# telespazio-tim/karios

Hardware: AMD Instinct MI355X
Metric: Mpixels/sec (+ matched keypoints/sec), Sentinel-2 10980^2 pair, KLT + ZNCC (higher is better)
Workload: dtype u8/i32 stencils, f32 LK solve, f64 stretch + ZNCC; 1 GPU; BASELINE config 2: 4 distinct S2-sized pairs 10980x10980 u16 resident in HBM, one per step, 4 per batched submissio...; distinct_pairs_resident=4, contexts=1, klt=Laplacian k=7, maxCorners 20000, one tile, ZNCC of rows with score >= 0.4, parallelism=1 rank(s), each a stream of independent band pairs

## Files before the change

include/karios_hip.h:

```cpp
#ifndef KARIOS_HIP_H
#define KARIOS_HIP_H

#include <stddef.h>
#include <stdint.h>

#ifdef __cplusplus
extern "C" {
#endif

typedef struct km_ctx km_ctx;

enum { KM_U8 = 0, KM_U16 = 1, KM_I16 = 2, KM_F32 = 3, KM_F64 = 4, KM_I32 = 5, KM_U32 = 6 };

enum {
    KM_OK = 0,
    KM_E_ARG = -1,
    KM_E_HIP = -2,
    KM_E_NOMEM = -3,
    KM_E_UNSUPPORTED = -4,
    KM_E_NO_DEVICE = -5,
    KM_E_INTERNAL = -6,
    KM_E_NO_CONVERGENCE = -7,
    KM_E_CAPACITY = -8
};
// ... 27 lines not shown
#define KM_PATH_STAGE_FALLBACK 2
#define KM_PATH_SECOND_PASS 4
#define KM_PATH_PREFIX_GROWN 8
#define KM_PATH_SPEC_RETRY 16
#define KM_PATH_MM_EARLY 32

int km_version(void);
int km_ctx_create(int device, km_ctx **out);
int km_ctx_destroy(km_ctx *ctx);
const char *km_last_error(km_ctx *ctx);
int km_ctx_sync(km_ctx *ctx);
int km_set_profiling(km_ctx *ctx, int enable);
int km_set_option(km_ctx *ctx, const char *name, int value);
int km_is_dev_build(void);
int km_dev_counters(km_ctx *ctx, unsigned long long out[2]);
int km_get_stage_ms(km_ctx *ctx, float *out, int cap, int *n);
const char *km_stage_name(int i);
int km_get_klt_stats(km_ctx *ctx, km_klt_stats *out);

int km_dev_alloc(km_ctx *ctx, size_t bytes, void **dptr);
int km_dev_free(km_ctx *ctx, void *dptr);
int km_h2d(km_ctx *ctx, void *dst_dev, const void *src_host, size_t bytes);
int km_d2h(km_ctx *ctx, void *dst_host, const void *src_dev, size_t bytes);
int km_host_alloc(km_ctx *ctx, size_t bytes, void **hptr);
int km_host_free(km_ctx *ctx , void *hptr);
int km_upload_async(km_ctx *ctx, void *dst_dev, size_t dst_pitch, const void *src_host, size_t src_pitch,
                    size_t width_bytes, size_t rows);
int km_upload_wait(km_ctx *ctx);
int km_upload_check_stats(km_ctx *ctx, int64_t *armed, int64_t *missed);
int km_upload_mark(km_ctx *ctx, int *ticket);
// ... 246 lines not shown
```

karios_amd/_lib.py:

```python
from __future__ import annotations

import ctypes as C
import os
import threading

import numpy as np

_HERE = os.path.dirname(os.path.abspath(__file__))
LIB_PATH = os.environ.get("KARIOS_HIP_LIB") or os.path.join(_HERE, "libkarios_hip.so")

KM_U8, KM_U16, KM_I16, KM_F32 = 0, 1, 2, 3
_DTYPES = {np.dtype("uint8"): KM_U8, np.dtype("uint16"): KM_U16, np.dtype("int16"): KM_I16,
           np.dtype("float32"): KM_F32}


class KariosHipError(RuntimeError):

    code = None


class KltParams(C.Structure):
    _fields_ = [("max_corners", C.c_int32), ("block_size", C.c_int32), ("win_size", C.c_int32),
                ("max_level", C.c_int32), ("max_count", C.c_int32), ("ksize_mon", C.c_int32),
                ("ksize_ref", C.c_int32), ("invert_mon", C.c_int32), ("quality_level", C.c_double),
# ... 47 lines not shown
ECC_CONVERGED, ECC_SKIPPED, ECC_NO_CONVERGENCE = 0, 1, 2

_vp, _i, _d, _sz, _pd = C.c_void_p, C.c_int, C.c_double, C.c_ssize_t, C.POINTER(C.c_double)
_pi = C.POINTER(C.c_int)

SIGNATURES = {
    "km_version": (_i, []),
    "km_ctx_create": (_i, [_i, C.POINTER(_vp)]),
    "km_ctx_destroy": (_i, [_vp]),
    "km_last_error": (C.c_char_p, [_vp]),
    "km_ctx_sync": (_i, [_vp]),
    "km_set_profiling": (_i, [_vp, _i]),
    "km_set_option": (_i, [_vp, C.c_char_p, _i]),
    "km_is_dev_build": (_i, []),
    "km_dev_counters": (_i, [_vp, C.POINTER(C.c_uint64)]),
    "km_get_stage_ms": (_i, [_vp, C.POINTER(C.c_float), _i, _pi]),
    "km_stage_name": (C.c_char_p, [_i]),
    "km_get_klt_stats": (_i, [_vp, C.POINTER(KltStats)]),
    "km_dev_alloc": (_i, [_vp, C.c_size_t, C.POINTER(_vp)]),
    "km_dev_free": (_i, [_vp, _vp]),
    "km_h2d": (_i, [_vp, _vp, _vp, C.c_size_t]),
    "km_d2h": (_i, [_vp, _vp, _vp, C.c_size_t]),
    "km_host_alloc": (_i, [_vp, C.c_size_t, C.POINTER(_vp)]),
    "km_host_free": (_i, [_vp, _vp]),
    "km_upload_async": (_i, [_vp, _vp, C.c_size_t, _vp, C.c_size_t, C.c_size_t, C.c_size_t]),
    "km_upload_wait": (_i, [_vp]),
    "km_upload_check_stats": (_i, [_vp, C.POINTER(C.c_int64), C.POINTER(C.c_int64)]),
    "km_upload_mark": (_i, [_vp, _pi]),
    "km_upload_join": (_i, [_vp, _i]),
    "km_set_frame_sink": (_i, [_vp, _vp, C.c_size_t]),
# ... 268 lines not shown
        self.check(self.lib.km_get_klt_stats(self.handle, C.byref(s)), "km_get_klt_stats")
        return s

    def set_profiling(self, on: bool):
        self.check(self.lib.km_set_profiling(self.handle, int(bool(on))), "km_set_profiling")

    def upload_check_stats(self):
        a, m = C.c_int64(), C.c_int64()
        self.check(self.lib.km_upload_check_stats(self.handle, C.byref(a), C.byref(m)), "km_upload_check_stats")
        return int(a.value), int(m.value)

    def set_option(self, name: str, value: int):
        self.check(self.lib.km_set_option(self.handle, name.encode(), int(value)), "km_set_option")
        self.__dict__.setdefault("_options", {})[name] = int(value)

    def set_frame_sink(self, ptr: int | None, nbytes: int = 0, pitch: int = 0) -> None:
        self.check(self.lib.km_set_frame_sink_pitch(self.handle, C.c_void_p(ptr) if ptr else None, int(nbytes) if ptr else 0, int(pitch) if ptr else 0),
                   "km_set_frame_sink_pitch")
        self.__dict__["_frame_sink"] = (int(ptr), int(nbytes), int(pitch)) if ptr else (None, 0, 0)

    @property
    def frame_sink(self) -> tuple:
        return self.__dict__.get("_frame_sink", (None, 0, 0))

    def get_option(self, name: str, default: int = 0) -> int:
        return self.__dict__.get("_options", {}).get(name, default)

    def phase_info(self) -> tuple[int, float]:
        path, margin = C.c_int(), C.c_double()
        self.check(self.lib.km_phase_info(self.handle, C.byref(path), C.byref(margin)), "km_phase_info")
# ... 35 lines not shown
```

karios_amd/csrc/api.hip:

```cpp
#include "api_internal.hpp"
#include "fft64_plan.hpp"
#include <vector>

#include <dlfcn.h>

#include <cstdarg>
#include <cstdio>
#include <cstdlib>
#include <cstring>
#include <new>

static thread_local std::string g_last_error;

int km_fail(km_ctx *ctx, int code, const char *fmt, ...)
{
    char buf[1024];
    va_list ap;
    va_start(ap, fmt);
    vsnprintf(buf, sizeof buf, fmt, ap);
    va_end(ap);
    g_last_error = buf;
    if (ctx) ctx->err = buf;
    return code;
}
// ... 130 lines not shown
    if (strcmp(name, "mm_early") == 0) { c->opt_mm_early = value != 0; return KM_OK; }
    if (strcmp(name, "frame_mi") == 0) { c->opt_frame_mi = value != 0; return KM_OK; }
    if (strcmp(name, "frame_clip") == 0) { c->opt_frame_clip = value != 0; return KM_OK; }
    if (strcmp(name, "units_pipeline") == 0) {
        if (!value) { const int rf = km_units_flush(c); if (rf) return rf; }
        c->opt_units_pipeline = value != 0;
        return KM_OK;
    }
    if (strcmp(name, "key_cap") == 0) { c->opt_key_cap = value < 0 ? 0 : value; return KM_OK; }
    if (strcmp(name, "stage_cap") == 0) { c->opt_stage_cap = value < 0 ? 0 : value; return KM_OK; }
    if (strcmp(name, "topk_factor") == 0) { c->opt_topk_factor = value < 0 ? 0 : value; return KM_OK; }
    if (strcmp(name, "select_first") == 0) { c->opt_select_first = value < 0 ? 0 : value; return KM_OK; }
    if (strcmp(name, "stash_cap") == 0) { c->opt_stash_cap = value < 0 ? 0 : value; return KM_OK; }
    if (strcmp(name, "spec_flag") == 0) { c->opt_spec_flag = value < 0 ? 0 : value; return KM_OK; }
    if (strcmp(name, "ransac_first_batch") == 0) { c->opt_ransac_first_batch = value < 0 ? 0 : value; return KM_OK; }
    if (strcmp(name, "defer") == 0) { c->opt_no_defer = value == 0; return KM_OK; }
    if (strcmp(name, "phase_fp64") == 0) { c->opt_phase_fp64 = value != 0; return KM_OK; }
    if (strcmp(name, "fft61") == 0) { c->opt_fft61 = value != 0; return KM_OK; }
    if (strcmp(name, "fft_herm") == 0) { c->opt_fft_herm = value != 0; return KM_OK; }
    if (strcmp(name, "f64_half") == 0) { c->opt_f64_half = value != 0; return KM_OK; }
    if (strcmp(name, "f64_pair") == 0) { c->opt_f64_pair = value != 0; return KM_OK; }
    if (strcmp(name, "f64_plain") == 0) { c->opt_f64_plain = value != 0; return KM_OK; }
    if (strcmp(name, "roctx") == 0) { c->opt_roctx = value != 0; return KM_OK; }
    if (strcmp(name, "profile_every") == 0) { c->opt_profile_every = value < 1 ? 1 : value; return KM_OK; }
    if (strcmp(name, "profile_stage") == 0) { c->opt_profile_stage = (value >= 0 && value < ST_COUNT) ? value : -1; return KM_OK; }
#ifdef KM_DEV
    if (strcmp(name, "fft_cross") == 0) { c->opt_fft_cross_fused = value != 0; return KM_OK; }
    if (strcmp(name, "f64_prime_t") == 0) { c->opt_f64_prime_t = value < 0 ? 0 : value; return KM_OK; }
    if (strcmp(name, "f64_smooth_t") == 0) { c->opt_f64_smooth_t = value < 0 ? 0 : value; return KM_OK; }
    if (strcmp(name, "defer_valid") == 0) { c->opt_defer_valid = value != 0; return KM_OK; }
    if (strcmp(name, "aux_early") == 0) { c->opt_aux_early = value != 0; return KM_OK; }
    if (strcmp(name, "aux_priority") == 0) { c->opt_aux_priority = value != 0; return KM_OK; }
    if (strcmp(name, "eig3_count") == 0) { c->opt_eig3_count = value != 0; return KM_OK; }
    if (strcmp(name, "prep_hist_plain") == 0) { c->opt_prep_plain = value != 0; return KM_OK; }
#endif
    return km_fail(c, KM_E_ARG, "km_set_option: unknown option '%s'", name);
}

int km_dev_counters(km_ctx *c, unsigned long long out[2])
{
#ifdef KM_DEV
    if (!c || !out) return km_fail(c, KM_E_ARG, "km_dev_counters: null argument");
    km_scalars *sc = (km_scalars *)c->ws[WS_SCALARS].p;
    if (!sc) return km_fail(c, KM_E_ARG, "km_dev_counters: no tile call yet");
    unsigned long long h[2];
    { const int rq = km_d2h_queue(c, h, &sc->skip_total, sizeof h); if (rq) return rq; }
    { const int rq = km_d2h_flush(c); if (rq) return rq; }
    out[0] = h[0]; out[1] = h[1];
    return KM_OK;
#else
    (void)out;
    return km_fail(c, KM_E_UNSUPPORTED, "km_dev_counters: development build only");
#endif
// ... 319 lines not shown
```

karios_amd/csrc/api_band.hip:

```cpp
#include "api_internal.hpp"

#include <cstring>
#include <vector>

extern "C" {

int km_minmax_dev(km_ctx *c, const void *d_img, int dtype, int H, int W, ptrdiff_t stride, double out_minmax[2])
{
    int rc;
    if ((rc = begin_call(c)) || (rc = check_image(c, d_img, H, W, stride, "minmax"))) return rc;
    if (!km_dtype_size(dtype) || !out_minmax) return km_fail(c, KM_E_ARG, "minmax: bad dtype %d or null output", dtype);
    km_scalars *sc = scalars(c);
    if (!sc) return KM_E_NOMEM;
    if (dtype == KM_U8) { out_minmax[0] = out_minmax[1] = 0.0; return KM_OK; }
    if ((rc = kd_minmax(c, d_img, dtype, H, W, stride, sc->mm))) return rc;
    KM_D2H(c, out_minmax, sc->mm, 2 * sizeof(double));
    KM_FLUSH(c);
    return KM_OK;
}

int km_band_prefilter_dev(km_ctx *c, const void *d_ref, const void *d_mon, int dtype, int H, int W, ptrdiff_t sref, ptrdiff_t smon,
                          const double minmax[4], const double *nodata_ref, const double *nodata_mon, int ksize_ref, int ksize_mon, int invert_mon,
                          int own_y0, int own_y1, const uint8_t *d_user_mask, uint8_t *d_lap_ref, uint8_t *d_lap_mon, uint8_t *d_mask,
                          int64_t *valid_owned)
{
    int rc;
    if ((rc = begin_call(c)) || (rc = check_image(c, d_ref, H, W, sref, "band_prefilter")) || (rc = check_image(c, d_mon, H, W, smon, "band_prefilter")))
        return rc;
    if (!km_dtype_size(dtype) || !minmax || !d_lap_ref || !d_lap_mon || !d_mask || !valid_owned) return km_fail(c, KM_E_ARG, "band_prefilter: bad arguments");
    if (own_y0 < 0 || own_y1 > H || own_y0 > own_y1) return km_fail(c, KM_E_ARG, "band_prefilter: own rows [%d, %d) outside 0..%d", own_y0, own_y1, H);
    km_scalars *sc = scalars(c);
    if (!sc) return KM_E_NOMEM;
    KM_HIP(c, hipMemsetAsync(sc, 0, sizeof *sc, c->stream));
    { const int rch = h2d_now(c, sc->mm, minmax, 4 * sizeof(double)); if (rch) return rch; }
    if ((rc = kd_stretch_laplacian_pair(c, d_ref, d_mon, dtype, H, W, sref, smon, sc->mm, ksize_ref, ksize_mon, invert_mon, nodata_ref, nodata_mon,
                                        d_lap_ref, d_lap_mon, d_user_mask ? nullptr : d_mask, &sc->valid)))
        return rc;
    if (d_user_mask) KM_HIP(c, hipMemcpyAsync(d_mask, d_user_mask, (size_t)H * W, hipMemcpyDeviceToDevice, c->stream));
    if (own_y0 > 0) KM_HIP(c, hipMemsetAsync(d_mask, 0, (size_t)own_y0 * W, c->stream));
    if (own_y1 < H) KM_HIP(c, hipMemsetAsync(d_mask + (size_t)own_y1 * W, 0, (size_t)(H - own_y1) * W, c->stream));
    KM_HIP(c, hipMemsetAsync(&sc->valid, 0, sizeof sc->valid, c->stream));
    if ((rc = kd_count_nonzero(c, d_mask, (size_t)H * W, &sc->valid))) return rc;
    unsigned long long v = 0;
    KM_D2H(c, &v, &sc->valid, sizeof v);
    KM_FLUSH(c);
    *valid_owned = (int64_t)v;
    return KM_OK;
}

int km_band_eigen_dev(km_ctx *c, const uint8_t *d_lap_ref, const uint8_t *d_mask, int H, int W, int block, double quality, unsigned *local_max_key)
{
    int rc;
// ... 176 lines not shown
```

karios_amd/csrc/common.hpp:

```cpp
#pragma once
#include <hip/hip_runtime.h>
#include <stddef.h>
#include <stdint.h>
#include <stdlib.h>
#include <atomic>
#include <memory>
#include <mutex>
#include <functional>
#include <string>
#include <vector>

#include "../../include/karios_hip.h"

#define KM_WAVE 64
#define KM_NSHARD 16
#define KM_TK_NB 2048
#define KM_UNITS_MAX 16

__host__ __device__ __forceinline__ int km_reflect101(int p, int len)
{
    if ((unsigned)p < (unsigned)len) return p;
    if (len == 1) return 0;
    do {
        p = p < 0 ? -p : 2 * len - 2 - p;
    } while ((unsigned)p >= (unsigned)len);
    return p;
}

enum km_stage {
    ST_MINMAX = 0,
    ST_LAPLACIAN,
// ... 141 lines not shown
    WS_SF_REFINED,
    WS_SF_KP,
    WS_SF_DESC,
    WS_SF_PERM,
    WS_SF_OUT,
    WS_AC_IN,
    WS_AC_COLS,
    WS_AC_BSUM,
    WS_AC_STATE,
    WS_AC_PART,
    WS_AC_FLAG,
    WS_AC_SCAN,
    WS_AC_KEYS0,
    WS_AC_KEYS1,
    WS_CL_COLS,
    WS_COUNT
};

struct km_scalars {
    double mm[4];
    unsigned long long valid;
    unsigned int max_eig_key;
    unsigned int n_cand;
    int n_corners;
    int n_batches;
    float thr;
    float max_eig;
    unsigned long long argmax_key;
    unsigned int run_max_key;
    unsigned int pad0;
// ... 115 lines not shown
    unsigned profile_tick = 0;
    bool profile_skip = false;
    int opt_profile_stage = -1;
    int opt_stash_cap = 0;
    int opt_spec_flag = 0;
    bool opt_roctx = false;
    bool opt_fft_cross_fused = true;
    bool opt_fft_herm = true;
    bool opt_fft61 = true;
    bool opt_phase_fp64 = false;
    bool opt_lk2 = true;
    bool opt_mm_early = true;
    bool opt_frame_mi = false;
    bool opt_frame_clip = false;
    int opt_ransac_first_batch = 0;
    bool opt_no_defer = false;
    km_event_h evs[KM_FRAME_SLOTS + 1][ST_COUNT][2];
    bool evs_used[KM_FRAME_SLOTS + 1][ST_COUNT];
    int ev_cur = 0;
    bool ev_ready = false;
    km_frame_slot fslot[KM_FRAME_SLOTS];
    int fslot_next = 0;
    km_pinned_mem pinned_rb;
    km_klt_stats stats;
    int phase_path = 0;
    double phase_margin = 0.0;
    bool opt_eig3_count = false;
    bool opt_prep_plain = false;
    bool opt_defer_valid = true;
    int f64_h = 0, f64_w = 0;
// ... 289 lines not shown
```

karios_amd/csrc/k_lap.hip:

```cpp
#include "k_pixel.hpp"
#include "lap_coef.hpp"

#include <algorithm>

#ifndef KM_LAPM_WAVES
#define KM_LAPM_WAVES 0
#endif
#if KM_LAPM_WAVES
#define KM_LAPM_OCC __attribute__((amdgpu_waves_per_eu(KM_LAPM_WAVES, KM_LAPM_WAVES)))
#else
#define KM_LAPM_OCC
#endif

#define LAP_TW 128
#define LAP_TH 16

template <typename T> struct stretcher {
    double mn, range;
    bool deg;
    __device__ void init(const double *mm, int img, const uint8_t *) {
        if constexpr (sizeof(T) == 1) { mn = 0; range = 1; deg = false; }
        else { mn = mm[2 * img]; const double mx = mm[2 * img + 1]; range = mx - mn; deg = !(mx > mn); }
    }
    __device__ __forceinline__ unsigned operator()(T v, const uint8_t *) const { return stretch_u8<T>(v, mn, range, deg); }
};
template <typename T> struct stretcher_i16 {
    int mn_i;
    double c1, c0;
    __device__ void init(const double *mm, int img, const uint8_t *) {
        const double mn = mm[2 * img], mx = mm[2 * img + 1];
        mn_i = (int)mn;
        if (mx > mn) { const double r = mx - mn; c1 = 255.0 / r; c0 = 0.5 / r; }
        else { c1 = 0.0; c0 = 0.0; }
    }
    __device__ __forceinline__ unsigned operator()(T v, const uint8_t *) const {
        return (unsigned)(int)__fma_rn((double)((int)v - mn_i), c1, c0);
    }
};
template <> struct stretcher<uint16_t> : stretcher_i16<uint16_t> {};
template <> struct stretcher<int16_t> : stretcher_i16<int16_t> {};

template <int R, typename T, int NIMG, bool MASK>
__global__ __launch_bounds__(256) void lap_kernel(const T *__restrict__ img0, const T *__restrict__ img1, int H, int W,
                                                  ptrdiff_t stride0, ptrdiff_t stride1, const double *__restrict__ mm,
                                                  lap_coef cf, int invert1, nodata_t nd,
                                                  uint8_t *__restrict__ out0, uint8_t *__restrict__ out1,
                                                  uint8_t *__restrict__ mask_out, unsigned *__restrict__ valid_partial)
{
    using HT = typename std::conditional<(R <= 3), short, int>::type;
    constexpr int HX = (R + 3) & ~3;
    constexpr int TWH = LAP_TW + 2 * HX;
    constexpr int THH = LAP_TH + 2 * R;
// ... 234 lines not shown
                if (ox + 3 < W && (off & 3) == 0) *(uint32_t *)(outs[i] + off) = packed;
                else {
                    for (int k = 0; k < 4 && ox + k < W; k++) outs[i][off + k] = (uint8_t)(packed >> (8 * k));
                }
            }
        }
    }
}

template <typename T, int NIMG, bool MASK>
static int launch_lap(km_ctx *c, int R, const T *a, const T *b, int H, int W, ptrdiff_t sa, ptrdiff_t sb, const double *mm,
                      const lap_coef &cf, int invert1, const nodata_t &nd, uint8_t *oa, uint8_t *ob, uint8_t *mask,
                      unsigned long long *valid_out)
{
    dim3 grid((W + LAP_TW - 1) / LAP_TW, (H + LAP_TH - 1) / LAP_TH);
    unsigned *valid = nullptr;
    if (MASK) {
        valid = (unsigned *)km_ws(c, WS_PARTIAL, (size_t)grid.x * grid.y * sizeof(unsigned));
        if (!valid) return KM_E_NOMEM;
    }
#define KM_LAP_CASE(RR)                                                                                         \
    case RR:                                                                                                    \
        lap_kernel<RR, T, NIMG, MASK><<<grid, 256, 0, c->stream>>>(a, b, H, W, sa, sb, mm, cf, invert1, nd, oa, ob, \
                                                                   mask, valid);                               \
        break;
    switch (R) {
        KM_LAP_CASE(1)
        KM_LAP_CASE(2)
        KM_LAP_CASE(3)
        KM_LAP_CASE(4)
// ... 17 lines not shown
    asm("v_dot4_i32_i8 %0, %1, %2, %3" : "=v"(r) : "v"(bytes), "s"(coef_uniform), "v"(acc));
    return r;
}
__device__ __forceinline__ int dot2_seed0(int pair, int coef_uniform)
{
    int r;
    asm("v_dot2_i32_i16 %0, %1, %2, 0" : "=v"(r) : "v"(pair), "s"(coef_uniform));
    return r;
}
__device__ __forceinline__ unsigned opaque_lane_offset(unsigned x)
{
    asm volatile("" : "+v"(x));
    return x;
}

#define LAPM_VALID_OF(R) ((R) == 5 ? 240 : 248)
#ifndef LAPM_PF
#define LAPM_PF 3
#endif

template <int R, typename T, bool MASK>
__device__ __forceinline__ void lap_march_item(const T *__restrict__ img0, const T *__restrict__ img1, int H, int W,
                                               ptrdiff_t stride0, ptrdiff_t stride1, const double *__restrict__ mm,
                                               const lap_coef &cf, int invert1, const nodata_t &nd,
                                               uint8_t *__restrict__ out0, uint8_t *__restrict__ out1,
                                               uint8_t *__restrict__ mask_out, unsigned *__restrict__ valid_partial, int nstrips,
                                               int rows_per_item, int wave_id )
{
    typedef short short2v __attribute__((ext_vector_type(2)));
    constexpr int RH = R == 5 ? 4 : R;
    constexpr int NR = 2 * RH + 1;
    constexpr int HALO = R == 5 ? 8 : 4, VALID = 256 - 2 * HALO;
    static_assert(VALID == LAPM_VALID_OF(R), "strip geometry");
    const int lane = threadIdx.x & 63;
    const int rowblock = wave_id / nstrips, strip = wave_id - rowblock * nstrips;
    stretcher<T> st[2];
    st[0].init(mm, 0, nullptr); st[1].init(mm, 1, nullptr);
    const bool shifted = (W % 4 != 0) && strip == nstrips - 1 && W >= 256;
    const int gx0 = (shifted ? W - (256 - HALO) : strip * VALID - HALO) + 4 * lane;
    const int cnt_from = shifted ? (nstrips - 1) * VALID : 0;
    const uint32_t cnt_mask = gx0 >= cnt_from ? 0xffffffffu : gx0 + 4 <= cnt_from ? 0u : (0xffffffffu << (8 * (cnt_from - gx0)));
    const unsigned ugx = (unsigned)gx0;
    const unsigned ugx_load = RH == 4 ? (unsigned)min(max(gx0 < 0 ? -gx0 - 3 : gx0 >= W ? 2 * W - 5 - gx0 : gx0, 0), W - 4) : (unsigned)min(max(gx0, 0), W - 4);
    const unsigned edge_sel = RH == 4 ? ((gx0 < 0 || gx0 >= W) ? 0x00010203u : 0x03020100u)
                                      : (gx0 < 0 ? 0x01020300u : gx0 >= W ? 0x03000102u : 0x03020100u);
    const bool col_inside = gx0 >= 0 && gx0 + 3 < W;
    const bool vec0 = col_inside && (stride0 % 4 == 0) && ((uintptr_t)img0 % (4 * sizeof(T)) == 0);
    const bool vec1 = col_inside && (stride1 % 4 == 0) && ((uintptr_t)img1 % (4 * sizeof(T)) == 0);
    int rc[4];
#pragma unroll
    for (int k = 0; k < 4; k++) rc[k] = km_reflect101(gx0 + k, W);
    const bool out_lane = lane >= HALO / 4 && lane <= 63 - HALO / 4 && gx0 < W;
// ... 25 lines not shown
    typedef unsigned short ushort2v __attribute__((ext_vector_type(2)));
    auto nodata16 = [](int has, double v) -> uint32_t {
        if (!has || v != floor(v)) return 0u;
        if constexpr (std::is_signed<T>::value) { if (v < -32768.0 || v > 32767.0) return 0u; }
        else { if (v < 0.0 || v > 65535.0) return 0u; }
        const uint32_t x = (uint32_t)(uint16_t)(int)v;
        return x | (x << 16);
    };
    const uint32_t nd16_mon = nodata16(nd.has_mon, nd.mon), nd16_ref = nodata16(nd.has_ref, nd.ref);
    (void)nd16_mon; (void)nd16_ref;
    int vbias[2];
    asm volatile("v_mov_b32 %0, %1" : "=v"(vbias[0]) : "s"(bias[0]));
    asm volatile("v_mov_b32 %0, %1" : "=v"(vbias[1]) : "s"(bias[1]));
    unsigned cnt = 0;
    uint8_t *outs[2] = {out0, out1};
    auto march = [&](auto fast_tag) {
    constexpr bool FAST = decltype(fast_tag)::value;
    auto load_raw = [&](int m, T (&v)[2][4]) {
        const int r = km_reflect101(m, H);
        const T *r0 = img0 + (size_t)r * stride0, *r1 = img1 + (size_t)r * stride1;
        const unsigned lx = opaque_lane_offset(ugx_load * (unsigned)sizeof(T));
        if (FAST) {
            __builtin_memcpy(v[0], (const char *)r0 + lx, 4 * sizeof(T));
        } else if (vec0) {
            if constexpr (sizeof(T) == 1) { uint32_t q = *(const uint32_t *)(r0 + gx0); __builtin_memcpy(v[0], &q, 4); }
            else if constexpr (sizeof(T) == 2) { uint2 q = *(const uint2 *)(r0 + gx0); __builtin_memcpy(v[0], &q, 8); }
            else { uint4 q = *(const uint4 *)(r0 + gx0); __builtin_memcpy(v[0], &q, 16); }
        } else {
#pragma unroll
            for (int k = 0; k < 4; k++) v[0][k] = r0[rc[k]];
        }
        if (FAST) {
// ... 14 lines not shown
#pragma unroll
        for (int r = 0; r < 2; r++)
#pragma unroll
            for (int j = 0; j < 4; j++) hp[i][r][j] = 0;
    (void)hp;
    int ring[2][NR][4];
#pragma unroll
    for (int i = 0; i < 2; i++)
#pragma unroll
        for (int k = 0; k < NR; k++)
#pragma unroll
            for (int j = 0; j < 4; j++) ring[i][k][j] = 0;
    T nxt[LAPM_PF][2][4];
#pragma unroll
    for (int f = 0; f < LAPM_PF; f++) load_raw(min(y0 - R + f, y1 + R - 1), nxt[f]);
    for (int mbase = y0 - R; mbase < y1 + R; mbase += NR) {
#pragma unroll
        for (int k = 0; k < NR; k++) {
            const int m = mbase + k;
            if (m >= y1 + R) continue;
            T v[2][4];
#pragma unroll
            for (int i = 0; i < 2; i++)
#pragma unroll
                for (int j = 0; j < 4; j++) {
                    v[i][j] = nxt[0][i][j];
#pragma unroll
                    for (int f = 0; f + 1 < LAPM_PF; f++) nxt[f][i][j] = nxt[f + 1][i][j];
                }
            if (m + LAPM_PF < y1 + R) load_raw(m + LAPM_PF, nxt[LAPM_PF - 1]);
            if constexpr (MASK && FAST && sizeof(T) == 2) {
                if (m >= y0 && m < y1 && out_lane) {
                    uint2 qm, qr;
                    __builtin_memcpy(&qm, v[1], 8); __builtin_memcpy(&qr, v[0], 8);
                    auto nz2 = [&](uint32_t a, uint32_t b) {
                        ushort2v mn2 = __builtin_elementwise_min(
                            __builtin_elementwise_min(__builtin_bit_cast(ushort2v, a), __builtin_bit_cast(ushort2v, b)),
                            __builtin_elementwise_min(__builtin_bit_cast(ushort2v, a ^ nd16_mon), __builtin_bit_cast(ushort2v, b ^ nd16_ref)));
                        mn2 = __builtin_elementwise_min(mn2, (ushort2v)(1));
                        return __builtin_bit_cast(uint32_t, mn2);
                    };
                    const uint32_t mp = __builtin_amdgcn_perm(nz2(qm.y, qr.y), nz2(qm.x, qr.x), 0x06040200u);
                    cnt += (unsigned)__popc(mp & cnt_mask);
                    __builtin_memcpy((mask_out + (size_t)m * W) + opaque_lane_offset(ugx), &mp, 4);
                }
// ... 2 lines not shown
                    uint32_t mp = 0;
#pragma unroll
                    for (int j = 0; j < 4; j++) {
                        const bool ok = (gx0 + j < W) && px_valid<T>(v[1][j], v[0][j], nd);
                        mp |= (ok ? 1u : 0u) << (8 * j);
                        cnt += ok && gx0 + j >= cnt_from;
                    }
                    const size_t o = (size_t)m * W + gx0;
                    if (FAST) __builtin_memcpy(mask_out + o, &mp, 4);
                    else if (gx0 + 3 < W && (o & 3) == 0) *(uint32_t *)(mask_out + o) = mp;
                    else {
                        for (int j = 0; j < 4 && gx0 + j < W; j++) mask_out[o + j] = (uint8_t)((mp >> (8 * j)) & 1u);
                    }
                }
            }
#pragma unroll
            for (int i = 0; i < 2; i++) {
                uint32_t cw = 0;
#pragma unroll
                for (int j = 0; j < 4; j++) cw |= st[i](v[i][j], nullptr) << (8 * j);
                cw ^= (i == 1 && invert1) ? 0x7f7f7f7fu : 0x80808080u;
                if constexpr (FAST) cw = __builtin_amdgcn_perm(cw, cw, edge_sel);
                const uint32_t lw = (uint32_t)__builtin_amdgcn_update_dpp(0, (int)cw, 0x138, 0xf, 0xf, false);
                const uint32_t rw = (uint32_t)__builtin_amdgcn_update_dpp(0, (int)cw, 0x130, 0xf, 0xf, false);
#pragma unroll
                for (int o = 0; o < 4; o++) {
                    constexpr int dummy = 0; (void)dummy;
                    if constexpr (RH == 4) {
                        const int g0 = (int)__builtin_amdgcn_alignbyte(cw, lw, o), g1 = (int)__builtin_amdgcn_alignbyte(rw, cw, o),
                                  g2 = (int)__builtin_amdgcn_alignbyte(0u, rw, o);
                        const int vd = __builtin_amdgcn_sdot4(g0, kdp[i][0], __builtin_amdgcn_sdot4(g1, kdp[i][1], dot4_seed0(g2, kdp[i][2]), false), false);
                        const int vs = __builtin_amdgcn_sdot4(g0, ksp[i][0], __builtin_amdgcn_sdot4(g1, ksp[i][1], dot4_seed0(g2, ksp[i][2]), false), false);
                        ring[i][k][o] = (int)__builtin_amdgcn_perm((uint32_t)vs, (uint32_t)vd, 0x05040100u);
                        continue;
                    }
                    const int sft = 4 + o - R;
                    int g0, g1;
// ... 66 lines not shown
                        packed |= (uint32_t)min(max(acc, 0), 255) << (8 * o);
                    }
                    const size_t off = (size_t)y * W + gx0;
                    if (FAST) __builtin_memcpy((outs[i] + (size_t)y * W) + opaque_lane_offset(ugx), &packed, 4);
                    else if (gx0 + 3 < W && (off & 3) == 0) *(uint32_t *)(outs[i] + off) = packed;
                    else {
                        for (int j = 0; j < 4 && gx0 + j < W; j++) outs[i][off + j] = (uint8_t)(packed >> (8 * j));
                    }
                }
            }
            }
        }
    }
    };
    const bool fast = (W % 4 == 0) || shifted || (strip * VALID - HALO + 4 * 64 <= W);
    if (fast) march(std::true_type{});
    else march(std::false_type{});
    if constexpr (MASK) {
        const unsigned c64 = (unsigned)wave_sum_u64((unsigned long long)cnt);
        if (lane == 0) valid_partial[wave_id] = c64;
    }
}

struct lapm_units_args {
    const void *img0[KM_UNITS_MAX], *img1[KM_UNITS_MAX];
    ptrdiff_t s0[KM_UNITS_MAX], s1[KM_UNITS_MAX];
    const double *mm[KM_UNITS_MAX];
    uint8_t *out0[KM_UNITS_MAX], *out1[KM_UNITS_MAX], *mask[KM_UNITS_MAX];
    unsigned *valid[KM_UNITS_MAX];
    int H[KM_UNITS_MAX], W[KM_UNITS_MAX], nstrips[KM_UNITS_MAX];
    int item0[KM_UNITS_MAX + 1];
    int n, rows;
};
template <int R, typename T, bool MASK>
__global__ __launch_bounds__(256) KM_LAPM_OCC void lap_march_units_kernel(lapm_units_args U, lap_coef cf, int invert1, nodata_t nd)
{
    const int total = U.item0[U.n];
    unsigned tile;
    if (!km_xcd_tile((unsigned)(total + 3) / 4u, tile)) return;
    const int wave_lin = (int)tile * 4 + __builtin_amdgcn_readfirstlane(threadIdx.x >> 6);
    if (wave_lin >= total) return;
    int u = 0;
    while (u + 1 < U.n && wave_lin >= U.item0[u + 1]) u++;
    lap_march_item<R, T, MASK>((const T *)U.img0[u], (const T *)U.img1[u], U.H[u], U.W[u], U.s0[u], U.s1[u], U.mm[u], cf, invert1, nd, U.out0[u], U.out1[u],
                               U.mask[u], U.valid[u], U.nstrips[u], U.rows, wave_lin - U.item0[u]);
}

template <typename T, bool MASK>
static const void *lapm_kernel(int R)
{
    return R == 1 ? (const void *)lap_march_units_kernel<1, T, MASK> : R == 2 ? (const void *)lap_march_units_kernel<2, T, MASK>
         : R == 3 ? (const void *)lap_march_units_kernel<3, T, MASK> : R == 4 ? (const void *)lap_march_units_kernel<4, T, MASK>
         : (const void *)lap_march_units_kernel<5, T, MASK>;
}

static void lapm_items(km_ctx *c, int R, const void *fn, lapm_units_args &A)
{
    int wg_per_cu = 0;
    if (hipOccupancyMaxActiveBlocksPerMultiprocessor(&wg_per_cu, fn, 256, 0) != hipSuccess || wg_per_cu < 1) wg_per_cu = 4;
    int rows = km_pick_rows_units(A.H, A.nstrips, A.n, 2 * R, (long)c->n_cu * 4 * wg_per_cu, 32, 160);
    if (const char *e = km_dev_env("KARIOS_HIP_LAP_ROWS")) { const int v = atoi(e); if (v >= 8 && v <= 4096) rows = v; }
    A.rows = rows;
    A.item0[0] = 0;
    for (int u = 0; u < A.n; u++) A.item0[u + 1] = A.item0[u] + A.nstrips[u] * ((A.H[u] + rows - 1) / rows);
}

static int lapm_launch(km_ctx *c, const void *fn, const lapm_units_args &A, const lap_coef &cf, int invert1, const nodata_t &nd)
{
    void *args[] = {(void *)&A, (void *)&cf, (void *)&invert1, (void *)&nd};
    KM_HIP(c, hipLaunchKernel(fn, dim3(km_xcd_grid((unsigned)(A.item0[A.n] + 3) / 4u)), dim3(256), args, 0, c->stream));
    return KM_OK;
}

template <typename T, bool MASK>
static int launch_lap_march(km_ctx *c, int R, const T *a, const T *b, int H, int W, ptrdiff_t sa, ptrdiff_t sb, const double *mm,
                            const lap_coef &cf, int invert1, const nodata_t &nd, uint8_t *oa, uint8_t *ob,
                            uint8_t *mask, unsigned long long *valid_out, km_valid_job *defer)
{
    lapm_units_args A;
    A.n = 1;
    A.img0[0] = a; A.img1[0] = b; A.s0[0] = sa; A.s1[0] = sb; A.mm[0] = mm;
    A.out0[0] = oa; A.out1[0] = ob; A.mask[0] = mask; A.valid[0] = nullptr;
    A.H[0] = H; A.W[0] = W; A.nstrips[0] = (W + LAPM_VALID_OF(R) - 1) / LAPM_VALID_OF(R);
    const void *fn = lapm_kernel<T, MASK>(R);
    lapm_items(c, R, fn, A);
    const unsigned nitems = (unsigned)A.item0[1];
    if (MASK) {
        A.valid[0] = (unsigned *)km_ws(c, WS_LAP_VALID, ((size_t)nitems + 4) * sizeof(unsigned));
        if (!A.valid[0]) return KM_E_NOMEM;
    }
    if (int rc = lapm_launch(c, fn, A, cf, invert1, nd)) return rc;
    if (MASK) {
        if (defer) {
            defer->partial = A.valid[0]; defer->n = nitems; defer->out = valid_out;
        } else if (int rc = kd_sum_u32(c, A.valid[0], nitems, valid_out)) return rc;
    }
    return KM_OK;
}

int kd_run_valid_sum(km_ctx *c, km_valid_job *job)
{
// ... 56 lines not shown
    if ((threadIdx.x & 63) == 0) sh[threadIdx.x >> 6] = (unsigned)s;
    __syncthreads();
    if (threadIdx.x == 0) A.partial[u][blockIdx.x] = sh[0] + sh[1] + sh[2] + sh[3];
}

template <typename T>
static int launch_lap_march_units(km_ctx *c, int R, const km_units &U, const lap_coef &cf, int invert1, const nodata_t &nd, km_valid_units *job)
{
    lapm_units_args A;
    A.n = U.n;
    for (int u = 0; u < U.n; u++) {
        A.img0[u] = U.ref[u]; A.img1[u] = U.mon[u]; A.s0[u] = U.sref[u]; A.s1[u] = U.smon[u]; A.mm[u] = U.mm[u];
        A.out0[u] = U.lap_ref[u]; A.out1[u] = U.lap_mon[u]; A.mask[u] = U.mask[u];
        A.H[u] = U.H[u]; A.W[u] = U.W[u]; A.nstrips[u] = (U.W[u] + LAPM_VALID_OF(R) - 1) / LAPM_VALID_OF(R);
    }
    lapm_items(c, R, lapm_kernel<T, true>(R), A);
    const int total = A.item0[U.n];
    const int mask_wgs = 256;
    const size_t n_partial = U.has_user_mask ? (size_t)mask_wgs * U.n : (size_t)total + 4 * KM_UNITS_MAX;
    unsigned *valid = (unsigned *)km_ws(c, WS_LAP_VALID, n_partial * sizeof(unsigned));
    if (!valid) return KM_E_NOMEM;
    job->n = U.n;
    if (U.has_user_mask) {
        mask_units_args M;
        for (int u = 0; u < U.n; u++) {
            M.src[u] = U.user_mask[u]; M.dst[u] = U.mask[u]; M.stride[u] = U.user_smask[u]; M.H[u] = U.H[u]; M.W[u] = U.W[u];
            M.partial[u] = valid + (size_t)mask_wgs * u;
            A.valid[u] = nullptr;
            job->partial[u] = M.partial[u]; job->n_partial[u] = (unsigned)mask_wgs; job->out[u] = &U.sc[u]->valid;
        }
        mask_pack_units_kernel<<<dim3(mask_wgs, U.n), 256, 0, c->stream>>>(M);
        KM_LAUNCH_CHECK(c);
        return lapm_launch(c, lapm_kernel<T, false>(R), A, cf, invert1, nd);
    }
    for (int u = 0; u < U.n; u++) {
        A.valid[u] = valid + A.item0[u];
        job->partial[u] = A.valid[u]; job->n_partial[u] = (unsigned)(A.item0[u + 1] - A.item0[u]); job->out[u] = &U.sc[u]->valid;
    }
    return lapm_launch(c, lapm_kernel<T, true>(R), A, cf, invert1, nd);
}

enum lap_form { LAP_NOT_COVERED = 0, LAP_GENERAL, LAP_MARCH };
struct lap_plan {
    int R = 0;
    lap_coef cf;
    lap_form form = LAP_NOT_COVERED;
};
static lap_plan lap_make_plan(int ksize_ref, int ksize_mon, int min_W, int min_H)
{
    lap_plan p;
    if (!km_lap_ksize_ok(ksize_ref) || !km_lap_ksize_ok(ksize_mon)) return p;
    const int ks[2] = {ksize_ref, ksize_mon};
// ... 49 lines not shown
```

Before: 147,400 Mpx/s.

## Use LDS lookup table for u16 contrast stretch in Laplacian march kernel

For 16-bit inputs, each workgroup precomputes the stretch-to-u8 mapping (with the invert/sign flip folded in) into LDS over the min..max range when it fits a byte budget. The march loop then replaces the per-pixel fp64 FMA with byte LDS lookups, prefetched one row ahead. Item counts are padded so every wave in a workgroup can reach the __syncthreads. Surplus waves help build the table and then exit. The change also adds a lap_rows option and a per-unit path word that records which path ran. The cost is up to 32 KB of dynamic LDS per workgroup, which may lower occupancy, plus a table-build prologue in every workgroup; the table is disabled on the single-band stretch path where min/max may not be exact.

```diff
diff --git a/include/karios_hip.h b/include/karios_hip.h
--- a/include/karios_hip.h
+++ b/include/karios_hip.h
@@ -65,6 +65,7 @@
 int km_set_option(km_ctx *ctx, const char *name, int value);
 int km_is_dev_build(void);
 int km_dev_counters(km_ctx *ctx, unsigned long long out[2]);
+int km_lap_table_paths(km_ctx *ctx, int *out, int cap, int *n);
 int km_get_stage_ms(km_ctx *ctx, float *out, int cap, int *n);
 const char *km_stage_name(int i);
 int km_get_klt_stats(km_ctx *ctx, km_klt_stats *out);
diff --git a/karios_amd/_lib.py b/karios_amd/_lib.py
--- a/karios_amd/_lib.py
+++ b/karios_amd/_lib.py
@@ -85,6 +85,7 @@
     "km_set_option": (_i, [_vp, C.c_char_p, _i]),
     "km_is_dev_build": (_i, []),
     "km_dev_counters": (_i, [_vp, C.POINTER(C.c_uint64)]),
+    "km_lap_table_paths": (_i, [_vp, C.POINTER(C.c_int), _i, C.POINTER(C.c_int)]),
     "km_get_stage_ms": (_i, [_vp, C.POINTER(C.c_float), _i, _pi]),
     "km_stage_name": (C.c_char_p, [_i]),
     "km_get_klt_stats": (_i, [_vp, C.POINTER(KltStats)]),
@@ -383,6 +384,11 @@
         self.check(self.lib.km_set_option(self.handle, name.encode(), int(value)), "km_set_option")
         self.__dict__.setdefault("_options", {})[name] = int(value)
 
+    def lap_table_paths(self) -> list:
+        out, n = (C.c_int * 16)(), C.c_int()
+        self.check(self.lib.km_lap_table_paths(self.handle, out, 16, C.byref(n)), "km_lap_table_paths")
+        return [int(out[u]) for u in range(min(int(n.value), 16))]
+
     def set_frame_sink(self, ptr: int | None, nbytes: int = 0, pitch: int = 0) -> None:
         self.check(self.lib.km_set_frame_sink_pitch(self.handle, C.c_void_p(ptr) if ptr else None, int(nbytes) if ptr else 0, int(pitch) if ptr else 0),
                    "km_set_frame_sink_pitch")
diff --git a/karios_amd/csrc/api.hip b/karios_amd/csrc/api.hip
--- a/karios_amd/csrc/api.hip
+++ b/karios_amd/csrc/api.hip
@@ -168,6 +168,9 @@
     if (strcmp(name, "stash_cap") == 0) { c->opt_stash_cap = value < 0 ? 0 : value; return KM_OK; }
     if (strcmp(name, "spec_flag") == 0) { c->opt_spec_flag = value < 0 ? 0 : value; return KM_OK; }
     if (strcmp(name, "ransac_first_batch") == 0) { c->opt_ransac_first_batch = value < 0 ? 0 : value; return KM_OK; }
+    if (strcmp(name, "lap_table") == 0) { c->opt_lap_table = value != 0; return KM_OK; }
+    if (strcmp(name, "lap_table_bytes") == 0) { c->opt_lap_table_bytes = value < 0 ? 0 : value > KM_LAP_TABLE_MAX ? KM_LAP_TABLE_MAX : value; return KM_OK; }
+    if (strcmp(name, "lap_rows") == 0) { c->opt_lap_rows = value < 0 ? 0 : value; return KM_OK; }
     if (strcmp(name, "defer") == 0) { c->opt_no_defer = value == 0; return KM_OK; }
     if (strcmp(name, "phase_fp64") == 0) { c->opt_phase_fp64 = value != 0; return KM_OK; }
     if (strcmp(name, "fft61") == 0) { c->opt_fft61 = value != 0; return KM_OK; }
@@ -191,6 +194,20 @@
     return km_fail(c, KM_E_ARG, "km_set_option: unknown option '%s'", name);
 }
 
+int km_lap_table_paths(km_ctx *c, int *out, int cap, int *n_out)
+{
+    if (!c || !out || !n_out || cap < 0) return km_fail(c, KM_E_ARG, "km_lap_table_paths: bad arguments");
+    { const int rs = km_ctx_sync(c); if (rs) return rs; }
+    const int n = c->lap_path_n < cap ? c->lap_path_n : cap;
+    *n_out = c->lap_path_n;
+    if (n <= 0) return KM_OK;
+    unsigned h[KM_UNITS_MAX];
+    { const int rq = km_d2h_queue(c, h, c->lap_path_dev, (size_t)n * sizeof(unsigned)); if (rq) return rq; }
+    { const int rq = km_d2h_flush(c); if (rq) return rq; }
+    for (int u = 0; u < n; u++) out[u] = (int)h[u];
+    return KM_OK;
+}
+
 int km_dev_counters(km_ctx *c, unsigned long long out[2])
 {
 #ifdef KM_DEV
diff --git a/karios_amd/csrc/api_band.hip b/karios_amd/csrc/api_band.hip
--- a/karios_amd/csrc/api_band.hip
+++ b/karios_amd/csrc/api_band.hip
@@ -33,9 +33,11 @@
     if (!sc) return KM_E_NOMEM;
     KM_HIP(c, hipMemsetAsync(sc, 0, sizeof *sc, c->stream));
     { const int rch = h2d_now(c, sc->mm, minmax, 4 * sizeof(double)); if (rch) return rch; }
-    if ((rc = kd_stretch_laplacian_pair(c, d_ref, d_mon, dtype, H, W, sref, smon, sc->mm, ksize_ref, ksize_mon, invert_mon, nodata_ref, nodata_mon,
-                                        d_lap_ref, d_lap_mon, d_user_mask ? nullptr : d_mask, &sc->valid)))
-        return rc;
+    c->lap_mm_exact = false;
+    rc = kd_stretch_laplacian_pair(c, d_ref, d_mon, dtype, H, W, sref, smon, sc->mm, ksize_ref, ksize_mon, invert_mon, nodata_ref, nodata_mon,
+                                   d_lap_ref, d_lap_mon, d_user_mask ? nullptr : d_mask, &sc->valid);
+    c->lap_mm_exact = true;
+    if (rc) return rc;
     if (d_user_mask) KM_HIP(c, hipMemcpyAsync(d_mask, d_user_mask, (size_t)H * W, hipMemcpyDeviceToDevice, c->stream));
     if (own_y0 > 0) KM_HIP(c, hipMemsetAsync(d_mask, 0, (size_t)own_y0 * W, c->stream));
     if (own_y1 < H) KM_HIP(c, hipMemsetAsync(d_mask + (size_t)own_y1 * W, 0, (size_t)(H - own_y1) * W, c->stream));
diff --git a/karios_amd/csrc/common.hpp b/karios_amd/csrc/common.hpp
--- a/karios_amd/csrc/common.hpp
+++ b/karios_amd/csrc/common.hpp
@@ -15,6 +15,7 @@
 #define KM_WAVE 64
 #define KM_NSHARD 16
 #define KM_TK_NB 2048
+#define KM_LAP_TABLE_MAX 65024
 #define KM_UNITS_MAX 16
 
 __host__ __device__ __forceinline__ int km_reflect101(int p, int len)
@@ -186,6 +187,7 @@
     WS_AC_KEYS0,
     WS_AC_KEYS1,
     WS_CL_COLS,
+    WS_LAP_PATH,
     WS_COUNT
 };
 
@@ -331,6 +333,12 @@
     bool opt_frame_mi = false;
     bool opt_frame_clip = false;
     int opt_ransac_first_batch = 0;
+    bool opt_lap_table = true;
+    int opt_lap_table_bytes = 32768;
+    int opt_lap_rows = 0;
+    bool lap_mm_exact = true;
+    const unsigned *lap_path_dev = nullptr;
+    int lap_path_n = 0;
     bool opt_no_defer = false;
     km_event_h evs[KM_FRAME_SLOTS + 1][ST_COUNT][2];
     bool evs_used[KM_FRAME_SLOTS + 1][ST_COUNT];
diff --git a/karios_amd/csrc/k_lap.hip b/karios_amd/csrc/k_lap.hip
--- a/karios_amd/csrc/k_lap.hip
+++ b/karios_amd/csrc/k_lap.hip
@@ -25,17 +25,16 @@
     __device__ __forceinline__ unsigned operator()(T v, const uint8_t *) const { return stretch_u8<T>(v, mn, range, deg); }
 };
 template <typename T> struct stretcher_i16 {
-    int mn_i;
+    int mn_i, r_i;
     double c1, c0;
     __device__ void init(const double *mm, int img, const uint8_t *) {
         const double mn = mm[2 * img], mx = mm[2 * img + 1];
         mn_i = (int)mn;
-        if (mx > mn) { const double r = mx - mn; c1 = 255.0 / r; c0 = 0.5 / r; }
-        else { c1 = 0.0; c0 = 0.0; }
-    }
-    __device__ __forceinline__ unsigned operator()(T v, const uint8_t *) const {
-        return (unsigned)(int)__fma_rn((double)((int)v - mn_i), c1, c0);
-    }
+        if (mx > mn) { const double r = mx - mn; c1 = 255.0 / r; c0 = 0.5 / r; r_i = (int)r; }
+        else { c1 = 0.0; c0 = 0.0; r_i = 0; }
+    }
+    __device__ __forceinline__ unsigned of_delta(int d) const { return (unsigned)(int)__fma_rn((double)d, c1, c0); }
+    __device__ __forceinline__ unsigned operator()(T v, const uint8_t *) const { return of_delta((int)v - mn_i); }
 };
 template <> struct stretcher<uint16_t> : stretcher_i16<uint16_t> {};
 template <> struct stretcher<int16_t> : stretcher_i16<int16_t> {};
@@ -300,6 +299,7 @@
                       unsigned long long *valid_out)
 {
     dim3 grid((W + LAP_TW - 1) / LAP_TW, (H + LAP_TH - 1) / LAP_TH);
+    c->lap_path_n = 0;
     unsigned *valid = nullptr;
     if (MASK) {
         valid = (unsigned *)km_ws(c, WS_PARTIAL, (size_t)grid.x * grid.y * sizeof(unsigned));
@@ -347,6 +347,11 @@
     return x;
 }
 
+extern __shared__ __attribute__((aligned(16))) uint8_t lapm_tab[];
+typedef __attribute__((address_space(3))) const uint8_t lds_u8;
+__device__ __forceinline__ unsigned lapm_tab_lds() { return (unsigned)(uintptr_t)(lds_u8 *)lapm_tab; }
+#define LAPM_WAVES 4
+
 #define LAPM_VALID_OF(R) ((R) == 5 ? 240 : 248)
 #ifndef LAPM_PF
 #define LAPM_PF 3
@@ -358,7 +363,9 @@
                                                const lap_coef &cf, int invert1, const nodata_t &nd,
                                                uint8_t *__restrict__ out0, uint8_t *__restrict__ out1,
                                                uint8_t *__restrict__ mask_out, unsigned *__restrict__ valid_partial, int nstrips,
-                                               int rows_per_item, int wave_id )
+                                               int rows_per_item, int wave_id ,
+                                               bool live ,
+                                               int tab_bytes , unsigned *__restrict__ path_word)
 {
     typedef short short2v __attribute__((ext_vector_type(2)));
     constexpr int RH = R == 5 ? 4 : R;
@@ -369,6 +376,30 @@
     const int rowblock = wave_id / nstrips, strip = wave_id - rowblock * nstrips;
     stretcher<T> st[2];
     st[0].init(mm, 0, nullptr); st[1].init(mm, 1, nullptr);
+    constexpr bool CAN_TABLE = sizeof(T) == 2;
+    bool use_table = false;
+    unsigned tab_adj[2] = {0u, 0u};
+    if constexpr (CAN_TABLE) {
+        const int n0 = st[0].r_i + 1, n1 = st[1].r_i + 1, off1 = (n0 + 3) & ~3;
+        use_table = tab_bytes > 0 && n0 + n1 <= tab_bytes;
+        if (use_table) {
+#pragma unroll
+            for (int i = 0; i < 2; i++) {
+                const int n = i ? n1 : n0, base = i ? off1 : 0;
+                const uint32_t flip = (i == 1 && invert1) ? 0x7f7f7f7fu : 0x80808080u;
+                for (int d = 4 * (int)threadIdx.x; d < n; d += 4 * 64 * LAPM_WAVES) {
+                    uint32_t w = 0;
+#pragma unroll
+                    for (int j = 0; j < 4; j++) w |= st[i].of_delta(min(d + j, n - 1)) << (8 * j);
+                    *(uint32_t *)(lapm_tab + base + d) = w ^ flip;
+                }
+                tab_adj[i] = (unsigned)(st[i].mn_i - base) - lapm_tab_lds();
+            }
+            __syncthreads();
+        }
+    }
+    if (!live) return;
+    if (wave_id == 0 && lane == 0) *path_word = use_table ? 1u : 2u;
     const bool shifted = (W % 4 != 0) && strip == nstrips - 1 && W >= 256;
     const int gx0 = (shifted ? W - (256 - HALO) : strip * VALID - HALO) + 4 * lane;
     const int cnt_from = shifted ? (nstrips - 1) * VALID : 0;
@@ -424,8 +455,21 @@
     asm volatile("v_mov_b32 %0, %1" : "=v"(vbias[1]) : "s"(bias[1]));
     unsigned cnt = 0;
     uint8_t *outs[2] = {out0, out1};
-    auto march = [&](auto fast_tag) {
+    auto march = [&](auto fast_tag, auto table_tag) {
     constexpr bool FAST = decltype(fast_tag)::value;
+    constexpr bool TABLE = decltype(table_tag)::value;
+    auto table_row = [&](const T (&vv)[2][4], uint32_t (&cw2)[2]) {
+#pragma unroll
+        for (int i = 0; i < 2; i++) {
+            uint32_t b[4];
+#pragma unroll
+            for (int j = 0; j < 4; j++) b[j] = *(lds_u8 *)(uintptr_t)((unsigned)(int)vv[i][j] - tab_adj[i]);
+            uint32_t cw = __builtin_amdgcn_perm(__builtin_amdgcn_perm(b[3], b[2], 0x0c0c0400u), __builtin_amdgcn_perm(b[1], b[0], 0x0c0c0400u), 0x05040100u);
+            if constexpr (FAST) cw = __builtin_amdgcn_perm(cw, cw, edge_sel);
+            cw2[i] = cw;
+        }
+    };
+    (void)table_row;
     auto load_raw = [&](int m, T (&v)[2][4]) {
         const int r = km_reflect101(m, H);
         const T *r0 = img0 + (size_t)r * stride0, *r1 = img1 + (size_t)r * stride1;
@@ -470,6 +514,9 @@
     T nxt[LAPM_PF][2][4];
 #pragma unroll
     for (int f = 0; f < LAPM_PF; f++) load_raw(min(y0 - R + f, y1 + R - 1), nxt[f]);
+    uint32_t cw_next[2] = {0u, 0u};
+    if constexpr (TABLE) table_row(nxt[0], cw_next);
+    (void)cw_next;
     for (int mbase = y0 - R; mbase < y1 + R; mbase += NR) {
 #pragma unroll
         for (int k = 0; k < NR; k++) {
@@ -485,6 +532,8 @@
                     for (int f = 0; f + 1 < LAPM_PF; f++) nxt[f][i][j] = nxt[f + 1][i][j];
                 }
             if (m + LAPM_PF < y1 + R) load_raw(m + LAPM_PF, nxt[LAPM_PF - 1]);
+            uint32_t cw_row[2] = {cw_next[0], cw_next[1]};
+            (void)cw_row;
             if constexpr (MASK && FAST && sizeof(T) == 2) {
                 if (m >= y0 && m < y1 && out_lane) {
                     uint2 qm, qr;
@@ -517,13 +566,17 @@
                     }
                 }
             }
+            if constexpr (TABLE) table_row(nxt[0], cw_next);
 #pragma unroll
             for (int i = 0; i < 2; i++) {
                 uint32_t cw = 0;
-#pragma unroll
-                for (int j = 0; j < 4; j++) cw |= st[i](v[i][j], nullptr) << (8 * j);
-                cw ^= (i == 1 && invert1) ? 0x7f7f7f7fu : 0x80808080u;
-                if constexpr (FAST) cw = __builtin_amdgcn_perm(cw, cw, edge_sel);
+                if constexpr (TABLE) cw = cw_row[i];
+                else {
+#pragma unroll
+                    for (int j = 0; j < 4; j++) cw |= st[i](v[i][j], nullptr) << (8 * j);
+                    cw ^= (i == 1 && invert1) ? 0x7f7f7f7fu : 0x80808080u;
+                    if constexpr (FAST) cw = __builtin_amdgcn_perm(cw, cw, edge_sel);
+                }
                 const uint32_t lw = (uint32_t)__builtin_amdgcn_update_dpp(0, (int)cw, 0x138, 0xf, 0xf, false);
                 const uint32_t rw = (uint32_t)__builtin_amdgcn_update_dpp(0, (int)cw, 0x130, 0xf, 0xf, false);
 #pragma unroll
@@ -620,8 +673,14 @@
     }
     };
     const bool fast = (W % 4 == 0) || shifted || (strip * VALID - HALO + 4 * 64 <= W);
-    if (fast) march(std::true_type{});
-    else march(std::false_type{});
+    if constexpr (CAN_TABLE) {
+        if (use_table) {
+            if (fast) march(std::true_type{}, std::true_type{});
+            else march(std::false_type{}, std::true_type{});
+        } else if (fast) march(std::true_type{}, std::false_type{});
+        else march(std::false_type{}, std::false_type{});
+    } else if (fast) march(std::true_type{}, std::false_type{});
+    else march(std::false_type{}, std::false_type{});
     if constexpr (MASK) {
         const unsigned c64 = (unsigned)wave_sum_u64((unsigned long long)cnt);
         if (lane == 0) valid_partial[wave_id] = c64;
@@ -635,21 +694,22 @@
     uint8_t *out0[KM_UNITS_MAX], *out1[KM_UNITS_MAX], *mask[KM_UNITS_MAX];
     unsigned *valid[KM_UNITS_MAX];
     int H[KM_UNITS_MAX], W[KM_UNITS_MAX], nstrips[KM_UNITS_MAX];
-    int item0[KM_UNITS_MAX + 1];
-    int n, rows;
+    int item0[KM_UNITS_MAX + 1], live[KM_UNITS_MAX];
+    unsigned *path;
+    int n, rows, tab_bytes;
 };
 template <int R, typename T, bool MASK>
 __global__ __launch_bounds__(256) KM_LAPM_OCC void lap_march_units_kernel(lapm_units_args U, lap_coef cf, int invert1, nodata_t nd)
 {
     const int total = U.item0[U.n];
     unsigned tile;
-    if (!km_xcd_tile((unsigned)(total + 3) / 4u, tile)) return;
-    const int wave_lin = (int)tile * 4 + __builtin_amdgcn_readfirstlane(threadIdx.x >> 6);
-    if (wave_lin >= total) return;
+    if (!km_xcd_tile((unsigned)total / LAPM_WAVES, tile)) return;
+    const int wave_lin = (int)tile * LAPM_WAVES + __builtin_amdgcn_readfirstlane(threadIdx.x >> 6);
     int u = 0;
     while (u + 1 < U.n && wave_lin >= U.item0[u + 1]) u++;
     lap_march_item<R, T, MASK>((const T *)U.img0[u], (const T *)U.img1[u], U.H[u], U.W[u], U.s0[u], U.s1[u], U.mm[u], cf, invert1, nd, U.out0[u], U.out1[u],
-                               U.mask[u], U.valid[u], U.nstrips[u], U.rows, wave_lin - U.item0[u]);
+                               U.mask[u], U.valid[u], U.nstrips[u], U.rows, wave_lin - U.item0[u], wave_lin - U.item0[u] < U.live[u], U.tab_bytes,
+                               U.path + u);
 }
 
 template <typename T, bool MASK>
@@ -660,21 +720,36 @@
          : (const void *)lap_march_units_kernel<5, T, MASK>;
 }
 
+template <typename T>
+static int lap_table_budget(const km_ctx *c)
+{
+    return (sizeof(T) == 2 && c->opt_lap_table && c->lap_mm_exact) ? c->opt_lap_table_bytes : 0;
+}
+static size_t lapm_table_lds(int tab_bytes) { return tab_bytes > 0 ? (size_t)((tab_bytes + 3) & ~3) + 8 : 0; }
+
 static void lapm_items(km_ctx *c, int R, const void *fn, lapm_units_args &A)
 {
     int wg_per_cu = 0;
-    if (hipOccupancyMaxActiveBlocksPerMultiprocessor(&wg_per_cu, fn, 256, 0) != hipSuccess || wg_per_cu < 1) wg_per_cu = 4;
-    int rows = km_pick_rows_units(A.H, A.nstrips, A.n, 2 * R, (long)c->n_cu * 4 * wg_per_cu, 32, 160);
+    if (hipOccupancyMaxActiveBlocksPerMultiprocessor(&wg_per_cu, fn, 64 * LAPM_WAVES, lapm_table_lds(A.tab_bytes)) != hipSuccess || wg_per_cu < 1) wg_per_cu = 4;
+    int rows = km_pick_rows_units(A.H, A.nstrips, A.n, 2 * R, (long)c->n_cu * LAPM_WAVES * wg_per_cu, 32, 160);
     if (const char *e = km_dev_env("KARIOS_HIP_LAP_ROWS")) { const int v = atoi(e); if (v >= 8 && v <= 4096) rows = v; }
+    if (c->opt_lap_rows >= 8 && c->opt_lap_rows <= 4096) rows = c->opt_lap_rows;
     A.rows = rows;
     A.item0[0] = 0;
-    for (int u = 0; u < A.n; u++) A.item0[u + 1] = A.item0[u] + A.nstrips[u] * ((A.H[u] + rows - 1) / rows);
-}
-
-static int lapm_launch(km_ctx *c, const void *fn, const lapm_units_args &A, const lap_coef &cf, int invert1, const nodata_t &nd)
-{
+    for (int u = 0; u < A.n; u++) {
+        A.live[u] = A.nstrips[u] * ((A.H[u] + rows - 1) / rows);
+        A.item0[u + 1] = A.item0[u] + (A.live[u] + LAPM_WAVES - 1) / LAPM_WAVES * LAPM_WAVES;
+    }
+}
+
+static int lapm_launch(km_ctx *c, const void *fn, lapm_units_args &A, const lap_coef &cf, int invert1, const nodata_t &nd)
+{
+    c->lap_path_n = 0;
+    A.path = (unsigned *)km_ws(c, WS_LAP_PATH, KM_UNITS_MAX * sizeof(unsigned));
+    if (!A.path) return KM_E_NOMEM;
     void *args[] = {(void *)&A, (void *)&cf, (void *)&invert1, (void *)&nd};
-    KM_HIP(c, hipLaunchKernel(fn, dim3(km_xcd_grid((unsigned)(A.item0[A.n] + 3) / 4u)), dim3(256), args, 0, c->stream));
+    KM_HIP(c, hipLaunchKernel(fn, dim3(km_xcd_grid((unsigned)A.item0[A.n] / LAPM_WAVES)), dim3(64 * LAPM_WAVES), args, lapm_table_lds(A.tab_bytes), c->stream));
+    c->lap_path_dev = A.path; c->lap_path_n = A.n;
     return KM_OK;
 }
 
@@ -688,9 +763,10 @@
     A.img0[0] = a; A.img1[0] = b; A.s0[0] = sa; A.s1[0] = sb; A.mm[0] = mm;
     A.out0[0] = oa; A.out1[0] = ob; A.mask[0] = mask; A.valid[0] = nullptr;
     A.H[0] = H; A.W[0] = W; A.nstrips[0] = (W + LAPM_VALID_OF(R) - 1) / LAPM_VALID_OF(R);
+    A.tab_bytes = lap_table_budget<T>(c);
     const void *fn = lapm_kernel<T, MASK>(R);
     lapm_items(c, R, fn, A);
-    const unsigned nitems = (unsigned)A.item0[1];
+    const unsigned nitems = (unsigned)A.live[0];
     if (MASK) {
         A.valid[0] = (unsigned *)km_ws(c, WS_LAP_VALID, ((size_t)nitems + 4) * sizeof(unsigned));
         if (!A.valid[0]) return KM_E_NOMEM;
@@ -777,6 +853,7 @@
         A.out0[u] = U.lap_ref[u]; A.out1[u] = U.lap_mon[u]; A.mask[u] = U.mask[u];
         A.H[u] = U.H[u]; A.W[u] = U.W[u]; A.nstrips[u] = (U.W[u] + LAPM_VALID_OF(R) - 1) / LAPM_VALID_OF(R);
     }
+    A.tab_bytes = lap_table_budget<T>(c);
     lapm_items(c, R, lapm_kernel<T, true>(R), A);
     const int total = A.item0[U.n];
     const int mask_wgs = 256;
@@ -798,7 +875,7 @@
     }
     for (int u = 0; u < U.n; u++) {
         A.valid[u] = valid + A.item0[u];
-        job->partial[u] = A.valid[u]; job->n_partial[u] = (unsigned)(A.item0[u + 1] - A.item0[u]); job->out[u] = &U.sc[u]->valid;
+        job->partial[u] = A.valid[u]; job->n_partial[u] = (unsigned)A.live[u]; job->out[u] = &U.sc[u]->valid;
     }
     return lapm_launch(c, lapm_kernel<T, true>(R), A, cf, invert1, nd);
 }
```

Result: no change. 148,600 Mpx/s, median of 6 (+0.9%).
